# bitlayer-org/tap-stark

Measured on AMD Instinct MI355X. Metric: trace cells/sec (proofs/sec alongside), 2^20x64 BabyBear trace, higher is better.
Workload: dtype u32

## Files before the change

### tap-stark_amd/csrc/kernels.hpp

```cpp
#pragma once
#include <stdint.h>

#include "bb.hpp"
#include "context.hpp"

namespace ts {

struct ColMat {
    uint32_t* d = nullptr;
    uint64_t height = 0;
    uint32_t width = 0;
    uint64_t col_stride = 0;
};

void launch_build_twiddles(Context& ctx, uint32_t* W, uint32_t* Winv, unsigned log_size);
void launch_build_shift_tables(Context& ctx, uint32_t* lo, uint32_t* hi, uint32_t n_hi,
                               uint32_t n_cosets, uint32_t shift_mont, unsigned log_N,
                               unsigned log_blowup, uint32_t scale_mont);
const uint32_t* coset_scale_table(Context& ctx, unsigned log_n, unsigned log_blowup, uint32_t shift);
void launch_transpose_bitrev(Context& ctx, const uint32_t* src, uint32_t* dst, unsigned log_n,
                             uint32_t w, uint64_t dst_col_stride, uint32_t src_width = 0);
bool launch_transpose_bitrev_r16(Context& ctx, const uint32_t* src, uint32_t* dst, unsigned log_n, uint32_t w,
                                 uint64_t dst_col_stride, uint32_t src_width = 0);
void launch_transpose_plain(Context& ctx, const uint32_t* src, uint32_t* dst, uint64_t n, uint32_t w,
                            uint64_t dst_col_stride);
void launch_transpose_to_row_major(Context& ctx, const uint32_t* src, uint64_t col_stride,
                                   uint32_t* dst, uint64_t h, uint32_t w);
void coset_lde(Context& ctx, uint32_t* evals, uint64_t in_col_stride, uint32_t ncols, unsigned log_n,
               unsigned log_blowup, uint32_t shift, uint32_t* out, uint64_t out_col_stride,
               uint32_t beta0 = 0, uint32_t n_beta = 0, bool first_round_done = false,
               uint32_t* evals2 = nullptr, uint32_t shift2 = 0, uint32_t gw = 0);

constexpr int MAX_BATCH_MATS = 64;
struct LeafMats {
    const uint32_t* d[MAX_BATCH_MATS];
    uint64_t col_stride[MAX_BATCH_MATS];
    uint32_t width[MAX_BATCH_MATS];
    uint8_t row_shift[MAX_BATCH_MATS];
    uint32_t n_mats;
    uint32_t total_width;
    const uint32_t* const* cols;
};
void launch_leaf_hash(Context& ctx, const LeafMats& mats, uint64_t height, uint32_t* digests);
void launch_leaf_hash_ef_pairs(Context& ctx, const uint32_t* vec, uint64_t n_rows, uint32_t* digests);
struct DevChallenger;
bool launch_merkle_levels(Context& ctx, uint32_t* tree, unsigned log_leaves,
// ... 48 lines not shown
};
void launch_bary_dots(Context& ctx, const ColMat& m, unsigned log_n, const Ef* weights,
                      uint32_t n_points, Ef* out, BaryPending* pending = nullptr);
void launch_bary_finish(Context& ctx, BaryPending& pending);
struct ReduceArgs {
    Ef z_mont[2];
    Ef off_mont[2];
    Ef rys[2];
    uint32_t n_points;
    uint32_t accumulate;
};
void launch_reduce(Context& ctx, const ColMat& m, unsigned log_h, const uint32_t* d_alpha_pows_mont,
                   const ReduceArgs& args, Ef* ro);
struct FusedReduceArgs {
    Ef z_mont[2];
    Ef off_t[2];
    Ef k0, k1;
    const uint32_t* chunk_w;
    const uint32_t* chunk[MAX_QUOTIENT_CHUNKS];
    uint64_t chunk_stride;
    uint32_t n_chunks;
    uint64_t row0, rows;
};
void launch_reduce_fused(Context& ctx, const ColMat& trace, unsigned log_h,
                         const uint32_t* d_alpha_pows_mont, const FusedReduceArgs& args, Ef* ro);

void launch_fri_fold(Context& ctx, const Ef* in, uint64_t h, Ef beta_canonical, Ef* out,
                     uint32_t* next_digests);
void launch_fri_fold_dev(Context& ctx, const Ef* in, uint64_t h, const Ef* d_beta, Ef* out,
                         uint32_t* next_digests, uint64_t h_global = 0, uint64_t row0 = 0);
// ... 45 lines not shown
```

### tap-stark_amd/csrc/ntt_lde.hip

```cpp
#include "kernels.hpp"

namespace ts {

constexpr int LOG_M = 12;
constexpr int NT_MID = 512;
constexpr int chunk_threads(int lm) { return lm == 14 ? 512 : 256; }
constexpr int TILE_ELEMS = 8192;

__device__ __forceinline__ uint32_t pad(uint32_t i) { return i + (i >> 5); }
constexpr int padded(int n) { return n + (n >> 5); }

template <int K, bool INV, bool TOP>
__device__ __forceinline__ void radix_butterflies(uint32_t (&v)[1 << K], unsigned s_base, unsigned u0,
                                                  uint32_t c, uint32_t hi,
                                                  const uint32_t* __restrict__ W) {
    constexpr int R = 1 << K;
    if (!INV) {
#pragma unroll
        for (int d = 0; d < K; d++) {
            const int half = R >> (d + 1);
            const uint32_t* __restrict__ wp = W + ((1u << (s_base + u0 + d)) + (c << (u0 + d)) + (hi << d));
#pragma unroll
            for (int q = 0; q < R; q++) {
                if ((q & half) == 0) {
// ... 94 lines not shown
template <int NTH>
__device__ __forceinline__ void tile_inverse_rt(uint32_t* s, unsigned log_len, unsigned log_T,
                                                unsigned s_base, uint32_t c,
                                                const uint32_t* __restrict__ Winv) {
    if (log_len == 0) return;
    const unsigned nr = (log_len + 3) / 4, q = log_len / nr, rem = log_len % nr;
    unsigned u = log_len;
    for (int r = (int)nr - 1; r >= 0; r--) {
        const unsigned k = q + ((unsigned)r < rem ? 1u : 0u);
        u -= k;
        radix_round_rt<true, NTH>((int)k, s, log_len + log_T, u, s_base, c, Winv);
    }
}

template <int LM>
__device__ __forceinline__ void chunk_load(uint32_t* s, const uint32_t* __restrict__ g) {
    constexpr int NT = chunk_threads(LM);
    const uint4* g4 = reinterpret_cast<const uint4*>(g);
    uint4 v[(1 << LM) / 4 / NT];
#pragma unroll
    for (int k = 0; k < (1 << LM) / 4 / NT; k++) v[k] = g4[threadIdx.x + (uint32_t)k * NT];
#pragma unroll
    for (int k = 0; k < (1 << LM) / 4 / NT; k++) {
        const uint32_t i4 = threadIdx.x + (uint32_t)k * NT;
        const uint32_t a = 4 * i4 + (i4 >> 3);
        s[a] = v[k].x;
        s[a + 1] = v[k].y;
        s[a + 2] = v[k].z;
        s[a + 3] = v[k].w;
    }
    __syncthreads();
}
template <int LM, bool CANON>
__device__ __forceinline__ void chunk_store(const uint32_t* s, uint32_t* __restrict__ g) {
    constexpr int NT = chunk_threads(LM);
    uint4* g4 = reinterpret_cast<uint4*>(g);
// ... 13 lines not shown
    constexpr int NT = chunk_threads(LM);
    constexpr int K0 = LM == 12 ? 4 : 5;
    constexpr int K1 = LM == 14 ? 5 : 4;
    static_assert(K0 + K1 + 4 == LM, "chunk plan");
    if (!INV) {
        radix_round<K0, false, LM - K0, NT>(s, LM, 0, sb, c, W);
        radix_round<K1, false, 4, NT>(s, LM, K0, sb, c, W);
        radix_round<4, false, 0, NT>(s, LM, K0 + K1, sb, c, W);
    } else {
        if (!SKIP_R16) radix_round<4, true, 0, NT>(s, LM, K0 + K1, sb, c, W);
        radix_round<K1, true, 4, NT>(s, LM, K0, sb, c, W);
        radix_round<K0, true, LM - K0, NT>(s, LM, 0, sb, c, W);
    }
}

template <int LM, bool SKIP_R16 = false>
__global__ void __launch_bounds__(chunk_threads(LM))
k_intt_contig(uint32_t* __restrict__ data, uint64_t col_stride, unsigned log_n,
              const uint32_t* __restrict__ Winv, uint32_t* __restrict__ data2, uint32_t gw) {
    __shared__ uint32_t s[padded(1 << LM)];
    const uint32_t c = blockIdx.x;
    uint32_t* col = blockIdx.y < gw ? data + (uint64_t)blockIdx.y * col_stride
                                    : data2 + (uint64_t)(blockIdx.y - gw) * col_stride;
    uint32_t* g = col + ((uint64_t)c << LM);
    chunk_load<LM>(s, g);
    chunk_rounds<LM, true, SKIP_R16>(s, log_n - LM, c, Winv);
    chunk_store<LM, false>(s, g);
}

__global__ void __launch_bounds__(256)
k_transpose_bitrev_r16(const uint32_t* __restrict__ src, uint32_t* __restrict__ dst, unsigned log_n,
                       uint32_t w, uint64_t dst_col_stride, uint32_t src_width,
                       const uint32_t* __restrict__ Winv) {
    __shared__ uint32_t tile[64][65];
    const uint32_t p0 = blockIdx.x << 6;
    const uint32_t c0 = blockIdx.y * 64;
    const uint32_t tx = threadIdx.x & 63, ty = threadIdx.x >> 6;
    const uint32_t rb = bitrev32(p0, log_n);
    const uint64_t row_step = (uint64_t)src_width << (log_n - 6);
    uint32_t v[16];
// ... 9 lines not shown
#pragma unroll
    for (int q = 0; q < 16; q++) tile[16 * ty + q][tx] = v[q];
    __syncthreads();
    uint32_t t[16];
#pragma unroll
    for (int k = 0; k < 16; k++) t[k] = tile[tx][ty + 4 * k];
    uint32_t* dp = dst + (uint64_t)(c0 + ty) * dst_col_stride + p0 + tx;
#pragma unroll
    for (int k = 0; k < 16; k++)
        if (c0 + ty + 4 * k < w) dp[(uint64_t)(4 * k) * dst_col_stride] = t[k];
}

template <int LM, int CPW = 1>
__global__ void __launch_bounds__(chunk_threads(LM), CPW > 1 ? 4 : 1)
k_lde_fwd_contig(uint32_t* __restrict__ out, uint64_t out_col_stride, unsigned log_n,
                 const uint32_t* __restrict__ W) {
    __shared__ uint32_t s[padded(1 << LM)];
    constexpr int NT = chunk_threads(LM);
    constexpr int NV = (1 << LM) / 4 / NT;
    const uint32_t beta = blockIdx.z;
    uint32_t* col = out + (uint64_t)blockIdx.y * out_col_stride + ((uint64_t)beta << log_n);
    if constexpr (CPW == 1) {
        const uint32_t c = blockIdx.x;
        uint32_t* o = col + ((uint64_t)c << LM);
        chunk_load<LM>(s, o);
        chunk_rounds<LM, false>(s, log_n - LM, c, W);
        chunk_store<LM, true>(s, o);
    } else {
        const uint32_t c0 = blockIdx.x * CPW;
        uint4 v[NV];
        {
            const uint4* g4 = reinterpret_cast<const uint4*>(col + ((uint64_t)c0 << LM));
#pragma unroll
            for (int k = 0; k < NV; k++) v[k] = g4[threadIdx.x + (uint32_t)k * NT];
        }
// ... 16 lines not shown
                for (int k = 0; k < NV; k++) v[k] = g4[threadIdx.x + (uint32_t)k * NT];
            }
            chunk_rounds<LM, false>(s, log_n - LM, c, W);
            chunk_store<LM, true>(s, col + ((uint64_t)c << LM));
            __syncthreads();
        }
    }
}

template <int PLAN, int TILE = TILE_ELEMS, int NTM = NT_MID, int LM = LOG_M>
__global__ void __launch_bounds__(NTM)
k_lde_mid(const uint32_t* __restrict__ evals, uint64_t in_col_stride, uint32_t* __restrict__ out,
          uint64_t out_col_stride, unsigned log_n, unsigned log_len, unsigned log_T,
          unsigned row_shift, unsigned beta0, unsigned n_cosets, const uint32_t* __restrict__ W,
          const uint32_t* __restrict__ Winv, const uint32_t* __restrict__ scale_a,
          const uint32_t* __restrict__ evals2, const uint32_t* __restrict__ scale_b, uint32_t gw) {
    __shared__ uint32_t s[padded(TILE)];
    constexpr int PER_THREAD = TILE / NTM;
    if (PLAN == 1) {
        log_len = 8;
        log_T = 5;
    }
    const bool remap = PLAN == 0 && log_T < 5 && gridDim.x >= 8;
    uint32_t bx = remap ? (blockIdx.x & 7) * (gridDim.x >> 3) + (blockIdx.x >> 3) : blockIdx.x;
    uint32_t col_id = blockIdx.y;
    if constexpr (PLAN == 1) {
        const uint32_t ncols = gridDim.x >> (LM - 5);
        bx = (blockIdx.x & 31) + 32 * (blockIdx.x / (32 * ncols));
        col_id = (blockIdx.x >> 5) % ncols;
    }
    const uint32_t j2_0 = bx << log_T;
    const uint32_t* g = (col_id < gw ? evals + (uint64_t)col_id * in_col_stride
                                     : evals2 + (uint64_t)(col_id - gw) * in_col_stride) + j2_0;
    const uint32_t* __restrict__ scale = col_id < gw ? scale_a : scale_b;
    const uint32_t total = 1u << (log_len + log_T);
    const uint32_t tmask = (1u << log_T) - 1;
    if constexpr (PLAN == 1) {
        uint32_t t[PER_THREAD];
#pragma unroll
        for (int k = 0; k < PER_THREAD; k++) {
            const uint32_t i = threadIdx.x + (uint32_t)k * NTM;
            t[k] = g[((uint64_t)(i >> log_T) << row_shift) + (i & tmask)];
        }
#pragma unroll
        for (int k = 0; k < PER_THREAD; k++) s[pad(threadIdx.x + (uint32_t)k * NTM)] = t[k];
    } else {
        for (uint32_t i = threadIdx.x; i < total; i += NTM)
            s[pad(i)] = g[((uint64_t)(i >> log_T) << row_shift) + (i & tmask)];
    }
    __syncthreads();
    if (PLAN == 1) {
        radix_round<4, true, 5, NTM>(s, 13, 4, 0, 0, Winv);
    } else {
        tile_inverse_rt<NTM>(s, log_len, log_T, 0, 0, Winv);
    }
    uint32_t coef[PER_THREAD];
#pragma unroll
    for (int k = 0; k < PER_THREAD; k++) {
        const uint32_t i = threadIdx.x + (uint32_t)k * NTM;
        coef[k] = i < total ? s[pad(i)] : 0u;
// ... 1 lines not shown
    constexpr int GP = PER_THREAD / 16;
    if constexpr (PLAN == 1) {
#pragma unroll
        for (int j = 0; j < GP; j++) {
            uint32_t v[16];
#pragma unroll
            for (int q = 0; q < 16; q++) v[q] = coef[j + GP * q];
            radix_butterflies<4, true, true>(v, 0, 0, 0, 0, Winv);
#pragma unroll
            for (int q = 0; q < 16; q++) coef[j + GP * q] = v[q];
        }
    }
    constexpr bool PREFETCH = PLAN == 1;
    uint32_t scv[PREFETCH ? 16 : 1];
    const uint32_t* scp = nullptr;
    if constexpr (PREFETCH) {
        const uint32_t i0 = threadIdx.x;
        scp = scale + ((uint64_t)(i0 >> 5) << LM) + (i0 & 31) + j2_0;
#pragma unroll
        for (int q = 0; q < 16; q++)
            scv[q] = (scp + ((uint64_t)beta0 << log_n))[(uint64_t)q * (NTM >> 5) << LM];
    }
    for (uint32_t bl = 0; bl < n_cosets; bl++) {
        const uint32_t beta = beta0 + bl;
        const uint32_t* sc = scale + ((uint64_t)beta << log_n);
        __syncthreads();
        if constexpr (PLAN == 1) {
#pragma unroll
            for (int j = 0; j < GP; j++) {
                uint32_t v[16];
#pragma unroll
                for (int q = 0; q < 16; q++) v[q] = mont_mul_lazy(coef[j + GP * q], scv[q]);
                if (bl + 1 < n_cosets) {
                    const uint32_t* nx = scp + ((uint64_t)(beta + 1) << log_n);
#pragma unroll
                    for (int q = 0; q < 16; q++) scv[q] = nx[(uint64_t)q * (NTM >> 5) << LM];
                }
                radix_butterflies<4, false, true>(v, 0, 0, 0, 0, W);
#pragma unroll
                for (int q = 0; q < 16; q++) s[pad(threadIdx.x + (uint32_t)(j + GP * q) * NTM)] = v[q];
            }
            __syncthreads();
            uint32_t* og = out + (uint64_t)col_id * out_col_stride + ((uint64_t)bl << log_n) + j2_0;
            radix_round<4, false, 5, NTM>(s, 13, 4, 0, 0, W);
            uint32_t t[PER_THREAD];
#pragma unroll
            for (int k = 0; k < PER_THREAD; k++) t[k] = s[pad(threadIdx.x + (uint32_t)k * NTM)];
            uint32_t* ot = og + ((uint64_t)(threadIdx.x >> 5) << LM) + (threadIdx.x & 31);
#pragma unroll
// ... 27 lines not shown
}

bool launch_transpose_bitrev_r16(Context& ctx, const uint32_t* src, uint32_t* dst, unsigned log_n, uint32_t w,
                                 uint64_t dst_col_stride, uint32_t src_width) {
    if (w == 0 || log_n <= lde_chunk_log(log_n)) return false;
    ctx.ensure_twiddles(log_n);
    TS_LAUNCH(ctx, k_transpose_bitrev_r16, dim3(1u << (log_n - 6), (w + 63) / 64), dim3(256), 0, src, dst, log_n, w,
              dst_col_stride, src_width ? src_width : w, (const uint32_t*)ctx.d_twiddle_inv);
    TS_HIP(hipGetLastError());
    return true;
}

void coset_lde(Context& ctx, uint32_t* evals, uint64_t in_col_stride, uint32_t ncols, unsigned log_n,
               unsigned log_blowup, uint32_t shift, uint32_t* out, uint64_t out_col_stride,
               uint32_t beta0, uint32_t n_beta, bool first_round_done, uint32_t* evals2, uint32_t shift2,
               uint32_t gw) {
    if (ncols == 0) return;
    TS_REQUIRE(evals2 == nullptr || (gw >= 1 && gw < ncols && shift2 != 0), TS_ERR_INVALID,
               "coset_lde: second matrix needs its first column and its shift");
    if (evals2 == nullptr) gw = 0xffffffffu;
    TS_REQUIRE(log_n + log_blowup <= 27, TS_ERR_INVALID, "coset_lde: log_n + log_blowup > 27");
    TS_REQUIRE(ncols >= 1 && ncols <= 65535, TS_ERR_INVALID, "coset_lde: bad column count");
    const unsigned LM = lde_chunk_log(log_n);
    TS_REQUIRE(!first_round_done || log_n > LM, TS_ERR_INVARIANT, "coset_lde: no contiguous inverse pass at this size");
    const bool two_pass = log_n > LM;
    const unsigned sA = two_pass ? log_n - LM : 0;
    TS_REQUIRE(sA <= 14, TS_ERR_INVALID, "coset_lde: log_n > 26");
    ctx.ensure_twiddles(log_n == 0 ? 1 : log_n);
    const uint32_t* W = ctx.d_twiddle_fwd;
    const uint32_t* Winv = ctx.d_twiddle_inv;
    unsigned log_T = 0;
    if (two_pass && sA <= 13)
        while ((1u << (sA + log_T + 1)) <= (unsigned)TILE_ELEMS && log_T < 6) log_T++;

    const uint32_t n_cosets = 1u << log_blowup;
    if (n_beta == 0) n_beta = n_cosets - beta0;
    TS_REQUIRE(beta0 < n_cosets && n_beta <= n_cosets - beta0, TS_ERR_INVALID, "coset_lde: coset range");
    const uint32_t* scale = coset_scale_table(ctx, log_n, log_blowup, shift);
    const uint32_t* scale2 = evals2 ? coset_scale_table(ctx, log_n, log_blowup, shift2) : nullptr;

    if (two_pass) {
        TS_REQUIRE(in_col_stride % 4 == 0 && out_col_stride % 4 == 0, TS_ERR_INVALID,
                   "coset_lde: column strides must be multiples of 4 elements");
        if (ctx.lde_pass_mask & 1u) {
            StageTimer t(&ctx, "lde: inverse NTT, contiguous stages");
            const dim3 g(1u << sA, ncols);
#define TS_INTT(LMV)                                                                                          \
    do {                                                                                                      \
        if (first_round_done)                                                                                 \
            TS_LAUNCH(ctx, (k_intt_contig<LMV, true>), g, dim3(chunk_threads(LMV)), 0, evals, in_col_stride, log_n, \
                      Winv, evals2, gw);                                                                      \
        else                                                                                                  \
            TS_LAUNCH(ctx, k_intt_contig<LMV>, g, dim3(chunk_threads(LMV)), 0, evals, in_col_stride, log_n, Winv, \
                      evals2, gw);                                                                            \
    } while (0)
            if (LM == 12) TS_INTT(12);
            else if (LM == 13) TS_INTT(13);
            else TS_INTT(14);
#undef TS_INTT
        }
        StageTimer t_rest(&ctx, "lde: strided pass + forward NTT of the owned cosets");
        const dim3 grid(1u << (LM - log_T), ncols);
        const dim3 grid1((1u << (LM - log_T)) * ncols);
#define TS_MID_ARGS                                                                            \
    (const uint32_t*)evals, in_col_stride, out, out_col_stride, log_n, sA, log_T, (unsigned)LM, \
        beta0, n_beta, W, Winv, scale, (const uint32_t*)evals2, scale2, gw
        if (!(ctx.lde_pass_mask & 2u)) {
        } else if (sA == 14)
            TS_LAUNCH(ctx, (k_lde_mid<0, 16384>), grid, dim3(NT_MID), 0, TS_MID_ARGS);
        else if (sA == 8 && log_T == 5 && LM == 12)
            TS_LAUNCH(ctx, k_lde_mid<1>, grid1, dim3(NT_MID), 0, TS_MID_ARGS);
        else if (sA == 8 && log_T == 5 && LM == 13)
            TS_LAUNCH(ctx, (k_lde_mid<1, 8192, 512, 13>), grid1, dim3(NT_MID), 0, TS_MID_ARGS);
        else if (sA == 8 && log_T == 5 && LM == 14)
            TS_LAUNCH(ctx, (k_lde_mid<1, 8192, 512, 14>), grid1, dim3(NT_MID), 0, TS_MID_ARGS);
        else
            TS_LAUNCH(ctx, k_lde_mid<0>, grid, dim3(NT_MID), 0, TS_MID_ARGS);
        const dim3 gf(1u << sA, ncols, n_beta);
        if (!(ctx.lde_pass_mask & 4u)) {
        } else if (LM == 12)
            TS_LAUNCH(ctx, k_lde_fwd_contig<12>, gf, dim3(chunk_threads(12)), 0, out, out_col_stride, log_n, W);
        else if (LM == 13)
            TS_LAUNCH(ctx, k_lde_fwd_contig<13>, gf, dim3(chunk_threads(13)), 0, out, out_col_stride, log_n, W);
        else
            TS_LAUNCH(ctx, (k_lde_fwd_contig<14, 4>), dim3(gf.x / 4, gf.y, gf.z), dim3(chunk_threads(14)), 0, out,
                      out_col_stride, log_n, W);
    } else {
        TS_LAUNCH(ctx, k_lde_mid<0>, dim3(1, ncols), dim3(NT_MID), 0, (const uint32_t*)evals,
                  in_col_stride, out, out_col_stride, log_n, log_n, 0u, 0u, beta0, n_beta, W, Winv, scale,
                  (const uint32_t*)evals2, scale2, gw);
    }
    TS_HIP(hipGetLastError());
}

}
```

### tap-stark_amd/csrc/open.hip

```cpp
#include "kernels.hpp"

namespace ts {

__device__ __forceinline__ uint32_t root_bitrev(const uint32_t* __restrict__ W, unsigned L, uint64_t r) {
    if (L == 0) return R_MOD_P;
    uint32_t w = W[((uint64_t)1 << (L - 1)) + (r >> 1)];
    return (r & 1) ? neg(w) : w;
}

constexpr int BW_ROWS = 4;

__global__ void __launch_bounds__(256)
k_bary_weights(unsigned log_n, const uint32_t* __restrict__ W, uint32_t gen_mont, Ef z0, Ef z1,
               uint32_t n_points, Ef* __restrict__ out) {
    const uint64_t n = 1ull << log_n;
    const uint64_t t0 = ((uint64_t)blockIdx.x * blockDim.x + threadIdx.x) * BW_ROWS;
    if (t0 >= n) return;
    Ef num[2 * BW_ROWS];
    uint32_t nrm[2 * BW_ROWS], pre[2 * BW_ROWS], xs[BW_ROWS];
    uint32_t run = R_MOD_P;
#pragma unroll
    for (int k = 0; k < BW_ROWS; k++) {
        const bool ok = t0 + k < n;
        uint32_t x = ok ? mont_mul(gen_mont, root_bitrev(W, log_n, t0 + k)) : R_MOD_P;
// ... 184 lines not shown
            TS_LAUNCH(ctx, (k_bary_dots<1, 64>), grid, dim3(256), 0, md, m.col_stride, m.width, log_n,
                      weights, partial.p, rows_per_block);
    }
    TS_HIP(hipGetLastError());
    BaryPending own;
    BaryPending& pend = pending ? *pending : own;
    if (pend.n == 2) launch_bary_finish(ctx, pend);
    pend.partial[pend.n] = std::move(partial);
    pend.out[pend.n] = reinterpret_cast<uint32_t*>(out);
    pend.n_blocks[pend.n] = n_blocks;
    pend.n_words[pend.n] = n_words;
    pend.n++;
    if (!pending) launch_bary_finish(ctx, pend);
}

__device__ __forceinline__ void row_dot_acc(uint64_t (&acc)[4], const uint32_t* __restrict__ m,
                                            uint64_t col_stride, uint32_t width, uint64_t X,
                                            const uint32_t* __restrict__ weights) {
    uint64_t a0 = acc[0], a1 = acc[1], a2 = acc[2], a3 = acc[3];
    constexpr int B = 8;
    const uint32_t* col = m + X;
    uint32_t i = 0;
    for (; i + B <= width; i += B) {
        uint32_t v[B];
#pragma unroll
        for (int k = 0; k < B; k++) v[k] = col[(uint64_t)(i + k) * col_stride];
#pragma unroll
        for (int k = 0; k < B; k++) {
            const uint32_t* ap = weights + 4 * (i + k);
            a0 = lazy_mac(a0, v[k], ap[0]);
            a1 = lazy_mac(a1, v[k], ap[1]);
            a2 = lazy_mac(a2, v[k], ap[2]);
            a3 = lazy_mac(a3, v[k], ap[3]);
            if (k & 1) {
                a0 = lazy_fix(a0);
                a1 = lazy_fix(a1);
                a2 = lazy_fix(a2);
                a3 = lazy_fix(a3);
            }
        }
    }
    if (i < width) {
        uint32_t v[B];
#pragma unroll
        for (int k = 0; k < B; k++) v[k] = i + k < width ? col[(uint64_t)(i + k) * col_stride] : 0u;
#pragma unroll
        for (int k = 0; k < B; k++) {
            if (i + k < width) {
                const uint32_t* ap = weights + 4 * (i + k);
                a0 = lazy_mac(a0, v[k], ap[0]);
                a1 = lazy_mac(a1, v[k], ap[1]);
                a2 = lazy_mac(a2, v[k], ap[2]);
                a3 = lazy_mac(a3, v[k], ap[3]);
            }
            if (k & 1) {
                a0 = lazy_fix(a0);
                a1 = lazy_fix(a1);
                a2 = lazy_fix(a2);
                a3 = lazy_fix(a3);
            }
        }
    }
    acc[0] = a0; acc[1] = a1; acc[2] = a2; acc[3] = a3;
}
__device__ __forceinline__ Ef row_dot_alpha(const uint32_t* __restrict__ m, uint64_t col_stride,
                                            uint32_t width, uint64_t X,
                                            const uint32_t* __restrict__ alpha_pows) {
    uint64_t acc[4] = {0, 0, 0, 0};
    row_dot_acc(acc, m, col_stride, width, X, alpha_pows);
    return Ef{{lazy_finish(acc[0]), lazy_finish(acc[1]), lazy_finish(acc[2]), lazy_finish(acc[3])}};
}

template <int NP>
__device__ __forceinline__ void inv_denoms(uint32_t x_mont, const Ef* z_mont, Ef* out) {
    Ef num[NP];
    uint32_t nrm[NP];
#pragma unroll
    for (int p = 0; p < NP; p++) {
        const Ef z = z_mont[p];
        Ef u = Ef{{sub(x_mont, z.c[0]), neg(z.c[1]), neg(z.c[2]), neg(z.c[3])}};
        ef_inv_parts(u, num[p], nrm[p]);
    }
    if (NP == 2) {
        uint32_t inv = mont_inv(mont_mul(nrm[0], nrm[NP - 1]));
        out[0] = ef_mul_base(num[0], mont_mul(inv, nrm[NP - 1]));
        out[NP - 1] = ef_mul_base(num[NP - 1], mont_mul(inv, nrm[0]));
    } else {
        out[0] = ef_mul_base(num[0], mont_inv(nrm[0]));
    }
}

template <int NP>
__global__ void __launch_bounds__(256)
k_reduce(const uint32_t* __restrict__ m, uint64_t col_stride, uint32_t width, unsigned log_h,
         const uint32_t* __restrict__ W, uint32_t gen_mont, const uint32_t* __restrict__ alpha_pows,
         ReduceArgs args, Ef* __restrict__ ro) {
    const uint64_t h = 1ull << log_h;
    const uint64_t X = (uint64_t)blockIdx.x * blockDim.x + threadIdx.x;
    if (X >= h) return;
    const Ef S = row_dot_alpha(m, col_stride, width, X, alpha_pows);
    const uint32_t x = mont_mul(gen_mont, root_bitrev(W, log_h, X));
    Ef inv_d[NP];
    inv_denoms<NP>(x, args.z_mont, inv_d);
// ... 11 lines not shown
    TS_REQUIRE(args.n_points >= 1 && args.n_points <= 2, TS_ERR_INVALID, "reduce: 1 or 2 points");
    ctx.ensure_twiddles(log_h == 0 ? 1 : log_h);
    const uint64_t h = 1ull << log_h;
    dim3 grid((unsigned)((h + 255) / 256));
    if (args.n_points == 2)
        TS_LAUNCH(ctx, k_reduce<2>, grid, dim3(256), 0, (const uint32_t*)m.d, m.col_stride, m.width,
                  log_h, (const uint32_t*)ctx.d_twiddle_fwd, to_mont(GENERATOR), d_alpha_pows_mont, args,
                  ro);
    else
        TS_LAUNCH(ctx, k_reduce<1>, grid, dim3(256), 0, (const uint32_t*)m.d, m.col_stride, m.width,
                  log_h, (const uint32_t*)ctx.d_twiddle_fwd, to_mont(GENERATOR), d_alpha_pows_mont, args,
                  ro);
    TS_HIP(hipGetLastError());
}

__global__ void __launch_bounds__(256)
k_reduce_fused(const uint32_t* __restrict__ trace, uint64_t trace_stride, uint32_t width,
               unsigned log_h, const uint32_t* __restrict__ W, uint32_t gen_mont,
               const uint32_t* __restrict__ alpha_pows, FusedReduceArgs a, Ef* __restrict__ ro) {
    const uint64_t X = (uint64_t)blockIdx.x * blockDim.x + threadIdx.x;
    if (X >= a.rows) return;
    const Ef St = row_dot_alpha(trace, trace_stride, width, X, alpha_pows);
    const uint32_t x = mont_mul(gen_mont, root_bitrev(W, log_h, a.row0 + X));
    Ef inv_d[2];
    inv_denoms<2>(x, a.z_mont, inv_d);
    uint64_t acc[4] = {0, 0, 0, 0};
    uint32_t c = 0;
    for (; c + 2 <= a.n_chunks; c += 2) {
        uint32_t v[8];
#pragma unroll
        for (int k = 0; k < 8; k++) v[k] = a.chunk[c + (k >> 2)][(uint64_t)(k & 3) * a.chunk_stride + X];
        const uint32_t* ap = a.chunk_w + 16 * c;
#pragma unroll
        for (int k = 0; k < 8; k++) {
#pragma unroll
            for (int j = 0; j < 4; j++) acc[j] = lazy_mac(acc[j], v[k], ap[4 * k + j]);
            if (k & 1) {
#pragma unroll
                for (int j = 0; j < 4; j++) acc[j] = lazy_fix(acc[j]);
            }
        }
    }
    for (; c < a.n_chunks; c++) row_dot_acc(acc, a.chunk[c], a.chunk_stride, 4, X, a.chunk_w + 16 * c);
    const Ef D{{lazy_finish(acc[0]), lazy_finish(acc[1]), lazy_finish(acc[2]), lazy_finish(acc[3])}};
    const Ef g0 = ef_sub(ef_add(ef_mul(St, a.off_t[0]), D), a.k0);
    const Ef g1 = ef_sub(ef_mul(St, a.off_t[1]), a.k1);
    const Ef r = ef_add(ef_mul(g0, inv_d[0]), ef_mul(g1, inv_d[1]));
    *reinterpret_cast<uint4*>(ro + X) = make_uint4(r.c[0], r.c[1], r.c[2], r.c[3]);
}

void launch_reduce_fused(Context& ctx, const ColMat& trace, unsigned log_h,
                         const uint32_t* d_alpha_pows_mont, const FusedReduceArgs& args, Ef* ro) {
    TS_REQUIRE(args.n_chunks <= (uint32_t)MAX_QUOTIENT_CHUNKS, TS_ERR_INVALID, "reduce_fused: too many chunks");
    ctx.ensure_twiddles(log_h == 0 ? 1 : log_h);
    FusedReduceArgs a = args;
    if (a.rows == 0) {
        a.row0 = 0;
        a.rows = 1ull << log_h;
    }
    TS_REQUIRE(a.row0 + a.rows <= (1ull << log_h), TS_ERR_INVALID, "reduce_fused: row range");
    TS_LAUNCH(ctx, k_reduce_fused, dim3((unsigned)((a.rows + 255) / 256)), dim3(256), 0,
              (const uint32_t*)trace.d, trace.col_stride, trace.width, log_h,
              (const uint32_t*)ctx.d_twiddle_fwd, to_mont(GENERATOR), d_alpha_pows_mont, a, ro);
    TS_HIP(hipGetLastError());
}

}
```

### tap-stark_amd/csrc/prover_common.cpp

```cpp
#include <stdlib.h>
#include <string.h>

#include <optional>

#include "prover_internal.hpp"

namespace ts {

void h2d(Context& ctx, void* dst, const void* src, size_t bytes) {
    if (!bytes) return;
    const void* from = bytes <= (1u << 20) ? ctx.stage(src, bytes) : src;
    TS_HIP(hipMemcpyAsync(dst, from, bytes, hipMemcpyHostToDevice, ctx.stream));
}
void d2h_sync(Context& ctx, void* dst, const void* src, size_t bytes) {
    if (bytes) TS_HIP(hipMemcpyAsync(dst, src, bytes, hipMemcpyDeviceToHost, ctx.stream));
    ctx.sync();
}

unsigned log2_strict(uint64_t n) {
    unsigned k = 0;
    while ((1ull << k) < n) k++;
    TS_REQUIRE((1ull << k) == n, TS_ERR_INVALID, "height must be a power of two");
    return k;
}
// ... 78 lines not shown
    auto push_lde = [&](uint32_t* d, uint64_t rows, uint32_t width) {
        ColMat cm;
        cm.d = d;
        cm.height = rows;
        cm.width = width;
        cm.col_stride = rows;
        data.ldes.push_back(cm);
    };

    StageTimer t(&ctx, "coset_lde");
    const bool batched = same_height && evals.size() > 1;
    DevBuf<uint32_t> batch;
    if (batched) batch = DevBuf<uint32_t>(&ctx, total_w * lde_rows(evals[0].height));
    size_t batch_col = 0;
    static const bool pair_knob = [] { const char* e = getenv("TS_LDE_PAIR"); return !e || atoi(e) != 0; }();
    if (allow_pair && pair_knob && batched && evals.size() == 2 && evals[0].width == evals[1].width &&
        evals[0].layout == DeviceMatrix::COL_MAJOR_BITREV && evals[1].layout == DeviceMatrix::COL_MAJOR_BITREV) {
        const uint64_t n = evals[0].height, rows = lde_rows(n);
        const uint32_t w = evals[0].width;
        coset_lde(ctx, evals[0].buf.p, n, 2 * w, log2_strict(n), fri.log_blowup,
                  mul(GENERATOR, inv_canon(domain_shifts[0])), batch.p, rows, beta0, n_beta, false, evals[1].buf.p,
                  mul(GENERATOR, inv_canon(domain_shifts[1])), w);
        for (size_t i = 0; i < 2; i++) {
            push_lde(batch.p + i * (size_t)w * rows, rows, w);
            evals[i].buf.reset();
        }
        data.lde_storage.push_back(std::move(batch));
        return;
    }
    for (size_t i = 0; i < evals.size(); i++) {
        DeviceMatrix& m = evals[i];
        const uint64_t n = m.height, rows = lde_rows(n);
        const unsigned log_n = log2_strict(n);
        DevBuf<uint32_t> colmajor;
        uint32_t* ev = m.buf.p;
        bool r16 = false;
        if (m.layout == DeviceMatrix::ROW_MAJOR) {
// ... 2 lines not shown
            colmajor = DevBuf<uint32_t>(&ctx, (size_t)m.width * n);
            r16 = launch_transpose_bitrev_r16(ctx, m.buf.p, colmajor.p, log_n, m.width, n);
            if (!r16) launch_transpose_bitrev(ctx, m.buf.p, colmajor.p, log_n, m.width, n);
            ev = colmajor.p;
        }
        DevBuf<uint32_t> own;
        uint32_t* lde;
        if (batched) {
            lde = batch.p + batch_col * rows;
            batch_col += m.width;
        } else {
            own = DevBuf<uint32_t>(&ctx, (size_t)m.width * rows);
            lde = own.p;
        }
        coset_lde(ctx, ev, n, m.width, log_n, fri.log_blowup, mul(GENERATOR, inv_canon(domain_shifts[i])), lde,
                  rows, beta0, n_beta, r16);
        push_lde(lde, rows, m.width);
        if (!batched) data.lde_storage.push_back(std::move(own));
        m.buf.reset();
    }
    if (batched) data.lde_storage.push_back(std::move(batch));
}

Statement check_statement(const FriConfig& fri, const AirProgram& air, uint32_t trace_width, uint64_t degree,
                          size_t n_public_values) {
    TS_REQUIRE(trace_width == air.width, TS_ERR_INVALID, "prove: trace width != AIR width");
    TS_REQUIRE(n_public_values == air.n_public, TS_ERR_INVALID, "prove: wrong number of public values");
    Statement s;
    s.log_degree = log2_strict(degree);
    s.lqd = air.log_quotient_degree;
    s.qd = 1u << s.lqd;
// ... 230 lines not shown
```

Baseline: 25.00 billion.

## Skip recomputing LDE coset equal to input domain; process row pairs in fused reduce

In the coset LDE, when some output coset coincides with the original evaluation domain (shift times coset root equals one), the input evaluations are copied straight into that output block during the inverse NTT load. The forward NTT and scaling for that coset are then skipped. Separately, the fused opening-reduce kernel now handles two adjacent rows per thread. The rows share their denominator inverses, taken from x and -x through a single inversion of z^2 - x^2, and their trace loads are vectorised. The cost is more template variants and a more complex coset loop, and the two-row path only runs when alignment and parity conditions hold.

New measurement: 25.17 billion, median of 6. Within noise of the previous version (+0.7%).

```diff
diff --git a/tap-stark_amd/csrc/kernels.hpp b/tap-stark_amd/csrc/kernels.hpp
--- a/tap-stark_amd/csrc/kernels.hpp
+++ b/tap-stark_amd/csrc/kernels.hpp
@@ -29,7 +29,7 @@
 void coset_lde(Context& ctx, uint32_t* evals, uint64_t in_col_stride, uint32_t ncols, unsigned log_n,
                unsigned log_blowup, uint32_t shift, uint32_t* out, uint64_t out_col_stride,
                uint32_t beta0 = 0, uint32_t n_beta = 0, bool first_round_done = false,
-               uint32_t* evals2 = nullptr, uint32_t shift2 = 0, uint32_t gw = 0);
+               uint32_t* evals2 = nullptr, uint32_t shift2 = 0, uint32_t gw = 0, uint32_t known = 0);
 
 constexpr int MAX_BATCH_MATS = 64;
 struct LeafMats {
@@ -108,6 +108,7 @@
                    const ReduceArgs& args, Ef* ro);
 struct FusedReduceArgs {
     Ef z_mont[2];
+    Ef z2_mont[2];
     Ef off_t[2];
     Ef k0, k1;
     const uint32_t* chunk_w;
diff --git a/tap-stark_amd/csrc/ntt_lde.hip b/tap-stark_amd/csrc/ntt_lde.hip
--- a/tap-stark_amd/csrc/ntt_lde.hip
+++ b/tap-stark_amd/csrc/ntt_lde.hip
@@ -6,6 +6,11 @@
 constexpr int NT_MID = 512;
 constexpr int chunk_threads(int lm) { return lm == 14 ? 512 : 256; }
 constexpr int TILE_ELEMS = 8192;
+
+constexpr uint32_t NO_BLOCK = 0xffffffffu;
+struct KnownBlocks {
+    uint32_t a, b;
+};
 
 __device__ __forceinline__ uint32_t pad(uint32_t i) { return i + (i >> 5); }
 constexpr int padded(int n) { return n + (n >> 5); }
@@ -132,12 +137,18 @@
 }
 
 template <int LM>
-__device__ __forceinline__ void chunk_load(uint32_t* s, const uint32_t* __restrict__ g) {
+__device__ __forceinline__ void chunk_load(uint32_t* s, const uint32_t* __restrict__ g,
+                                           uint32_t* __restrict__ raw = nullptr) {
     constexpr int NT = chunk_threads(LM);
     const uint4* g4 = reinterpret_cast<const uint4*>(g);
     uint4 v[(1 << LM) / 4 / NT];
 #pragma unroll
     for (int k = 0; k < (1 << LM) / 4 / NT; k++) v[k] = g4[threadIdx.x + (uint32_t)k * NT];
+    if (raw) {
+        uint4* r4 = reinterpret_cast<uint4*>(raw);
+#pragma unroll
+        for (int k = 0; k < (1 << LM) / 4 / NT; k++) r4[threadIdx.x + (uint32_t)k * NT] = v[k];
+    }
 #pragma unroll
     for (int k = 0; k < (1 << LM) / 4 / NT; k++) {
         const uint32_t i4 = threadIdx.x + (uint32_t)k * NT;
@@ -181,16 +192,24 @@
     }
 }
 
-template <int LM, bool SKIP_R16 = false>
+template <int LM, bool SKIP_R16 = false, bool KNOWN = false>
 __global__ void __launch_bounds__(chunk_threads(LM))
 k_intt_contig(uint32_t* __restrict__ data, uint64_t col_stride, unsigned log_n,
-              const uint32_t* __restrict__ Winv, uint32_t* __restrict__ data2, uint32_t gw) {
+              const uint32_t* __restrict__ Winv, uint32_t* __restrict__ data2, uint32_t gw,
+              uint32_t* __restrict__ out, uint64_t out_col_stride, KnownBlocks kb) {
     __shared__ uint32_t s[padded(1 << LM)];
     const uint32_t c = blockIdx.x;
     uint32_t* col = blockIdx.y < gw ? data + (uint64_t)blockIdx.y * col_stride
                                     : data2 + (uint64_t)(blockIdx.y - gw) * col_stride;
     uint32_t* g = col + ((uint64_t)c << LM);
-    chunk_load<LM>(s, g);
+    if constexpr (KNOWN) {
+        const uint32_t k = blockIdx.y < gw ? kb.a : kb.b;
+        chunk_load<LM>(s, g, k == NO_BLOCK ? nullptr
+                                           : out + (uint64_t)blockIdx.y * out_col_stride + ((uint64_t)k << log_n) +
+                                                 ((uint64_t)c << LM));
+    } else {
+        chunk_load<LM>(s, g);
+    }
     chunk_rounds<LM, true, SKIP_R16>(s, log_n - LM, c, Winv);
     chunk_store<LM, false>(s, g);
 }
@@ -230,11 +249,12 @@
 template <int LM, int CPW = 1>
 __global__ void __launch_bounds__(chunk_threads(LM), CPW > 1 ? 4 : 1)
 k_lde_fwd_contig(uint32_t* __restrict__ out, uint64_t out_col_stride, unsigned log_n,
-                 const uint32_t* __restrict__ W) {
+                 const uint32_t* __restrict__ W, uint32_t gw, KnownBlocks kb) {
     __shared__ uint32_t s[padded(1 << LM)];
     constexpr int NT = chunk_threads(LM);
     constexpr int NV = (1 << LM) / 4 / NT;
     const uint32_t beta = blockIdx.z;
+    if (beta == (blockIdx.y < gw ? kb.a : kb.b)) return;
     uint32_t* col = out + (uint64_t)blockIdx.y * out_col_stride + ((uint64_t)beta << log_n);
     if constexpr (CPW == 1) {
         const uint32_t c = blockIdx.x;
@@ -281,7 +301,8 @@
           uint64_t out_col_stride, unsigned log_n, unsigned log_len, unsigned log_T,
           unsigned row_shift, unsigned beta0, unsigned n_cosets, const uint32_t* __restrict__ W,
           const uint32_t* __restrict__ Winv, const uint32_t* __restrict__ scale_a,
-          const uint32_t* __restrict__ evals2, const uint32_t* __restrict__ scale_b, uint32_t gw) {
+          const uint32_t* __restrict__ evals2, const uint32_t* __restrict__ scale_b, uint32_t gw,
+          KnownBlocks known) {
     __shared__ uint32_t s[padded(TILE)];
     constexpr int PER_THREAD = TILE / NTM;
     if (PLAN == 1) {
@@ -300,6 +321,7 @@
     const uint32_t* g = (col_id < gw ? evals + (uint64_t)col_id * in_col_stride
                                      : evals2 + (uint64_t)(col_id - gw) * in_col_stride) + j2_0;
     const uint32_t* __restrict__ scale = col_id < gw ? scale_a : scale_b;
+    const uint32_t kb = col_id < gw ? known.a : known.b;
     const uint32_t total = 1u << (log_len + log_T);
     const uint32_t tmask = (1u << log_T) - 1;
     if constexpr (PLAN == 1) {
@@ -311,6 +333,9 @@
         }
 #pragma unroll
         for (int k = 0; k < PER_THREAD; k++) s[pad(threadIdx.x + (uint32_t)k * NTM)] = t[k];
+    } else if (row_shift == 0 && kb != NO_BLOCK) {
+        uint32_t* ok = out + (uint64_t)col_id * out_col_stride + ((uint64_t)kb << log_n);
+        for (uint32_t i = threadIdx.x; i < total; i += NTM) s[pad(i)] = ok[i] = g[i];
     } else {
         for (uint32_t i = threadIdx.x; i < total; i += NTM)
             s[pad(i)] = g[((uint64_t)(i >> log_T) << row_shift) + (i & tmask)];
@@ -342,14 +367,18 @@
     constexpr bool PREFETCH = PLAN == 1;
     uint32_t scv[PREFETCH ? 16 : 1];
     const uint32_t* scp = nullptr;
+    const uint32_t bl0 = kb == 0 ? 1u : 0u;
     if constexpr (PREFETCH) {
         const uint32_t i0 = threadIdx.x;
         scp = scale + ((uint64_t)(i0 >> 5) << LM) + (i0 & 31) + j2_0;
-#pragma unroll
-        for (int q = 0; q < 16; q++)
-            scv[q] = (scp + ((uint64_t)beta0 << log_n))[(uint64_t)q * (NTM >> 5) << LM];
-    }
-    for (uint32_t bl = 0; bl < n_cosets; bl++) {
+        if (bl0 < n_cosets) {
+#pragma unroll
+            for (int q = 0; q < 16; q++)
+                scv[q] = (scp + ((uint64_t)(beta0 + bl0) << log_n))[(uint64_t)q * (NTM >> 5) << LM];
+        }
+    }
+    for (uint32_t bl = bl0, bl_next; bl < n_cosets; bl = bl_next) {
+        bl_next = bl + 1 == kb ? bl + 2 : bl + 1;
         const uint32_t beta = beta0 + bl;
         const uint32_t* sc = scale + ((uint64_t)beta << log_n);
         __syncthreads();
@@ -359,8 +388,8 @@
                 uint32_t v[16];
 #pragma unroll
                 for (int q = 0; q < 16; q++) v[q] = mont_mul_lazy(coef[j + GP * q], scv[q]);
-                if (bl + 1 < n_cosets) {
-                    const uint32_t* nx = scp + ((uint64_t)(beta + 1) << log_n);
+                if (bl_next < n_cosets) {
+                    const uint32_t* nx = scp + ((uint64_t)(beta0 + bl_next) << log_n);
 #pragma unroll
                     for (int q = 0; q < 16; q++) scv[q] = nx[(uint64_t)q * (NTM >> 5) << LM];
                 }
@@ -418,7 +447,7 @@
 void coset_lde(Context& ctx, uint32_t* evals, uint64_t in_col_stride, uint32_t ncols, unsigned log_n,
                unsigned log_blowup, uint32_t shift, uint32_t* out, uint64_t out_col_stride,
                uint32_t beta0, uint32_t n_beta, bool first_round_done, uint32_t* evals2, uint32_t shift2,
-               uint32_t gw) {
+               uint32_t gw, uint32_t known) {
     if (ncols == 0) return;
     TS_REQUIRE(evals2 == nullptr || (gw >= 1 && gw < ncols && shift2 != 0), TS_ERR_INVALID,
                "coset_lde: second matrix needs its first column and its shift");
@@ -442,6 +471,18 @@
     TS_REQUIRE(beta0 < n_cosets && n_beta <= n_cosets - beta0, TS_ERR_INVALID, "coset_lde: coset range");
     const uint32_t* scale = coset_scale_table(ctx, log_n, log_blowup, shift);
     const uint32_t* scale2 = evals2 ? coset_scale_table(ctx, log_n, log_blowup, shift2) : nullptr;
+    auto known_block = [&](uint32_t sh) {
+        const uint32_t w = two_adic_generator(log_n + log_blowup);
+        for (uint32_t bl = 0; bl < n_beta; bl++)
+            if (mul(sh, pow_canon(w, bitrev32(beta0 + bl, log_blowup))) == 1) return bl;
+        return NO_BLOCK;
+    };
+    KnownBlocks kb{NO_BLOCK, NO_BLOCK};
+    if (!first_round_done) {
+        if (known & 1u) kb.a = known_block(shift);
+        if (evals2 && (known & 2u)) kb.b = known_block(shift2);
+    }
+    const bool any_known = kb.a != NO_BLOCK || kb.b != NO_BLOCK;
 
     if (two_pass) {
         TS_REQUIRE(in_col_stride % 4 == 0 && out_col_stride % 4 == 0, TS_ERR_INVALID,
@@ -449,26 +490,28 @@
         if (ctx.lde_pass_mask & 1u) {
             StageTimer t(&ctx, "lde: inverse NTT, contiguous stages");
             const dim3 g(1u << sA, ncols);
+#define TS_INTT_ARGS evals, in_col_stride, log_n, Winv, evals2, gw, out, out_col_stride, kb
 #define TS_INTT(LMV)                                                                                          \
     do {                                                                                                      \
         if (first_round_done)                                                                                 \
-            TS_LAUNCH(ctx, (k_intt_contig<LMV, true>), g, dim3(chunk_threads(LMV)), 0, evals, in_col_stride, log_n, \
-                      Winv, evals2, gw);                                                                      \
+            TS_LAUNCH(ctx, (k_intt_contig<LMV, true>), g, dim3(chunk_threads(LMV)), 0, TS_INTT_ARGS);         \
+        else if (any_known)                                                                                   \
+            TS_LAUNCH(ctx, (k_intt_contig<LMV, false, true>), g, dim3(chunk_threads(LMV)), 0, TS_INTT_ARGS);  \
         else                                                                                                  \
-            TS_LAUNCH(ctx, k_intt_contig<LMV>, g, dim3(chunk_threads(LMV)), 0, evals, in_col_stride, log_n, Winv, \
-                      evals2, gw);                                                                            \
+            TS_LAUNCH(ctx, k_intt_contig<LMV>, g, dim3(chunk_threads(LMV)), 0, TS_INTT_ARGS);                 \
     } while (0)
             if (LM == 12) TS_INTT(12);
             else if (LM == 13) TS_INTT(13);
             else TS_INTT(14);
 #undef TS_INTT
+#undef TS_INTT_ARGS
         }
         StageTimer t_rest(&ctx, "lde: strided pass + forward NTT of the owned cosets");
         const dim3 grid(1u << (LM - log_T), ncols);
         const dim3 grid1((1u << (LM - log_T)) * ncols);
 #define TS_MID_ARGS                                                                            \
     (const uint32_t*)evals, in_col_stride, out, out_col_stride, log_n, sA, log_T, (unsigned)LM, \
-        beta0, n_beta, W, Winv, scale, (const uint32_t*)evals2, scale2, gw
+        beta0, n_beta, W, Winv, scale, (const uint32_t*)evals2, scale2, gw, kb
         if (!(ctx.lde_pass_mask & 2u)) {
         } else if (sA == 14)
             TS_LAUNCH(ctx, (k_lde_mid<0, 16384>), grid, dim3(NT_MID), 0, TS_MID_ARGS);
@@ -483,16 +526,16 @@
         const dim3 gf(1u << sA, ncols, n_beta);
         if (!(ctx.lde_pass_mask & 4u)) {
         } else if (LM == 12)
-            TS_LAUNCH(ctx, k_lde_fwd_contig<12>, gf, dim3(chunk_threads(12)), 0, out, out_col_stride, log_n, W);
+            TS_LAUNCH(ctx, k_lde_fwd_contig<12>, gf, dim3(chunk_threads(12)), 0, out, out_col_stride, log_n, W, gw, kb);
         else if (LM == 13)
-            TS_LAUNCH(ctx, k_lde_fwd_contig<13>, gf, dim3(chunk_threads(13)), 0, out, out_col_stride, log_n, W);
+            TS_LAUNCH(ctx, k_lde_fwd_contig<13>, gf, dim3(chunk_threads(13)), 0, out, out_col_stride, log_n, W, gw, kb);
         else
             TS_LAUNCH(ctx, (k_lde_fwd_contig<14, 4>), dim3(gf.x / 4, gf.y, gf.z), dim3(chunk_threads(14)), 0, out,
-                      out_col_stride, log_n, W);
+                      out_col_stride, log_n, W, gw, kb);
     } else {
         TS_LAUNCH(ctx, k_lde_mid<0>, dim3(1, ncols), dim3(NT_MID), 0, (const uint32_t*)evals,
                   in_col_stride, out, out_col_stride, log_n, log_n, 0u, 0u, beta0, n_beta, W, Winv, scale,
-                  (const uint32_t*)evals2, scale2, gw);
+                  (const uint32_t*)evals2, scale2, gw, kb);
     }
     TS_HIP(hipGetLastError());
 }
diff --git a/tap-stark_amd/csrc/open.hip b/tap-stark_amd/csrc/open.hip
--- a/tap-stark_amd/csrc/open.hip
+++ b/tap-stark_amd/csrc/open.hip
@@ -222,79 +222,118 @@
     if (!pending) launch_bary_finish(ctx, pend);
 }
 
-__device__ __forceinline__ void row_dot_acc(uint64_t (&acc)[4], const uint32_t* __restrict__ m,
+template <int R>
+__device__ __forceinline__ void load_rows(uint32_t (&v)[R], const uint32_t* __restrict__ p) {
+    if constexpr (R == 2) {
+        const uint2 t = *reinterpret_cast<const uint2*>(p);
+        v[0] = t.x;
+        v[1] = t.y;
+    } else {
+        v[0] = *p;
+    }
+}
+template <int R>
+__device__ __forceinline__ void row_dot_acc(uint64_t (&acc)[R][4], const uint32_t* __restrict__ m,
                                             uint64_t col_stride, uint32_t width, uint64_t X,
                                             const uint32_t* __restrict__ weights) {
-    uint64_t a0 = acc[0], a1 = acc[1], a2 = acc[2], a3 = acc[3];
     constexpr int B = 8;
     const uint32_t* col = m + X;
     uint32_t i = 0;
     for (; i + B <= width; i += B) {
-        uint32_t v[B];
-#pragma unroll
-        for (int k = 0; k < B; k++) v[k] = col[(uint64_t)(i + k) * col_stride];
+        uint32_t v[B][R];
+#pragma unroll
+        for (int k = 0; k < B; k++) load_rows<R>(v[k], col + (uint64_t)(i + k) * col_stride);
 #pragma unroll
         for (int k = 0; k < B; k++) {
             const uint32_t* ap = weights + 4 * (i + k);
-            a0 = lazy_mac(a0, v[k], ap[0]);
-            a1 = lazy_mac(a1, v[k], ap[1]);
-            a2 = lazy_mac(a2, v[k], ap[2]);
-            a3 = lazy_mac(a3, v[k], ap[3]);
-            if (k & 1) {
-                a0 = lazy_fix(a0);
-                a1 = lazy_fix(a1);
-                a2 = lazy_fix(a2);
-                a3 = lazy_fix(a3);
+#pragma unroll
+            for (int r = 0; r < R; r++) {
+#pragma unroll
+                for (int j = 0; j < 4; j++) acc[r][j] = lazy_mac(acc[r][j], v[k][r], ap[j]);
+                if (k & 1) {
+#pragma unroll
+                    for (int j = 0; j < 4; j++) acc[r][j] = lazy_fix(acc[r][j]);
+                }
             }
         }
     }
     if (i < width) {
-        uint32_t v[B];
-#pragma unroll
-        for (int k = 0; k < B; k++) v[k] = i + k < width ? col[(uint64_t)(i + k) * col_stride] : 0u;
+        uint32_t v[B][R];
 #pragma unroll
         for (int k = 0; k < B; k++) {
             if (i + k < width) {
-                const uint32_t* ap = weights + 4 * (i + k);
-                a0 = lazy_mac(a0, v[k], ap[0]);
-                a1 = lazy_mac(a1, v[k], ap[1]);
-                a2 = lazy_mac(a2, v[k], ap[2]);
-                a3 = lazy_mac(a3, v[k], ap[3]);
-            }
-            if (k & 1) {
-                a0 = lazy_fix(a0);
-                a1 = lazy_fix(a1);
-                a2 = lazy_fix(a2);
-                a3 = lazy_fix(a3);
-            }
-        }
-    }
-    acc[0] = a0; acc[1] = a1; acc[2] = a2; acc[3] = a3;
+                load_rows<R>(v[k], col + (uint64_t)(i + k) * col_stride);
+            } else {
+#pragma unroll
+                for (int r = 0; r < R; r++) v[k][r] = 0u;
+            }
+        }
+#pragma unroll
+        for (int k = 0; k < B; k++) {
+#pragma unroll
+            for (int r = 0; r < R; r++) {
+                if (i + k < width) {
+                    const uint32_t* ap = weights + 4 * (i + k);
+#pragma unroll
+                    for (int j = 0; j < 4; j++) acc[r][j] = lazy_mac(acc[r][j], v[k][r], ap[j]);
+                }
+                if (k & 1) {
+#pragma unroll
+                    for (int j = 0; j < 4; j++) acc[r][j] = lazy_fix(acc[r][j]);
+                }
+            }
+        }
+    }
+}
+__device__ __forceinline__ Ef lazy_finish_ef(const uint64_t (&acc)[4]) {
+    return Ef{{lazy_finish(acc[0]), lazy_finish(acc[1]), lazy_finish(acc[2]), lazy_finish(acc[3])}};
 }
 __device__ __forceinline__ Ef row_dot_alpha(const uint32_t* __restrict__ m, uint64_t col_stride,
                                             uint32_t width, uint64_t X,
                                             const uint32_t* __restrict__ alpha_pows) {
-    uint64_t acc[4] = {0, 0, 0, 0};
-    row_dot_acc(acc, m, col_stride, width, X, alpha_pows);
-    return Ef{{lazy_finish(acc[0]), lazy_finish(acc[1]), lazy_finish(acc[2]), lazy_finish(acc[3])}};
-}
-
+    uint64_t acc[1][4] = {{0, 0, 0, 0}};
+    row_dot_acc<1>(acc, m, col_stride, width, X, alpha_pows);
+    return lazy_finish_ef(acc[0]);
+}
+
+__device__ __forceinline__ void ef_inv_two(Ef u0, Ef u1, Ef& i0, Ef& i1) {
+    Ef num0, num1;
+    uint32_t nrm0, nrm1;
+    ef_inv_parts(u0, num0, nrm0);
+    ef_inv_parts(u1, num1, nrm1);
+    const uint32_t inv = mont_inv(mont_mul(nrm0, nrm1));
+    i0 = ef_mul_base(num0, mont_mul(inv, nrm1));
+    i1 = ef_mul_base(num1, mont_mul(inv, nrm0));
+}
 template <int NP>
 __device__ __forceinline__ void inv_denoms(uint32_t x_mont, const Ef* z_mont, Ef* out) {
-    Ef num[NP];
-    uint32_t nrm[NP];
+    Ef u[NP];
 #pragma unroll
     for (int p = 0; p < NP; p++) {
         const Ef z = z_mont[p];
-        Ef u = Ef{{sub(x_mont, z.c[0]), neg(z.c[1]), neg(z.c[2]), neg(z.c[3])}};
-        ef_inv_parts(u, num[p], nrm[p]);
-    }
-    if (NP == 2) {
-        uint32_t inv = mont_inv(mont_mul(nrm[0], nrm[NP - 1]));
-        out[0] = ef_mul_base(num[0], mont_mul(inv, nrm[NP - 1]));
-        out[NP - 1] = ef_mul_base(num[NP - 1], mont_mul(inv, nrm[0]));
+        u[p] = Ef{{sub(x_mont, z.c[0]), neg(z.c[1]), neg(z.c[2]), neg(z.c[3])}};
+    }
+    if constexpr (NP == 2) {
+        ef_inv_two(u[0], u[1], out[0], out[1]);
     } else {
-        out[0] = ef_mul_base(num[0], mont_inv(nrm[0]));
+        Ef num;
+        uint32_t nrm;
+        ef_inv_parts(u[0], num, nrm);
+        out[0] = ef_mul_base(num, mont_inv(nrm));
+    }
+}
+__device__ __forceinline__ void inv_denoms_pair(uint32_t x_mont, const Ef* z_mont, const Ef* z2_mont, Ef* pos,
+                                                Ef* neg_) {
+    const uint32_t xx = mont_mul(x_mont, x_mont);
+    Ef d[2], e[2];
+#pragma unroll
+    for (int p = 0; p < 2; p++) d[p] = Ef{{sub(z2_mont[p].c[0], xx), z2_mont[p].c[1], z2_mont[p].c[2], z2_mont[p].c[3]}};
+    ef_inv_two(d[0], d[1], e[0], e[1]);
+#pragma unroll
+    for (int p = 0; p < 2; p++) {
+        const Ef ze = ef_mul(z_mont[p], e[p]), xe = ef_mul_base(e[p], x_mont);
+        pos[p] = ef_neg(ef_add(xe, ze));
+        neg_[p] = ef_sub(xe, ze);
     }
 }
 
@@ -336,39 +375,58 @@
     TS_HIP(hipGetLastError());
 }
 
+template <int R>
 __global__ void __launch_bounds__(256)
 k_reduce_fused(const uint32_t* __restrict__ trace, uint64_t trace_stride, uint32_t width,
                unsigned log_h, const uint32_t* __restrict__ W, uint32_t gen_mont,
                const uint32_t* __restrict__ alpha_pows, FusedReduceArgs a, Ef* __restrict__ ro) {
-    const uint64_t X = (uint64_t)blockIdx.x * blockDim.x + threadIdx.x;
+    const uint64_t X = ((uint64_t)blockIdx.x * blockDim.x + threadIdx.x) * R;
     if (X >= a.rows) return;
-    const Ef St = row_dot_alpha(trace, trace_stride, width, X, alpha_pows);
+    uint64_t acc[R][4];
+#pragma unroll
+    for (int r = 0; r < R; r++)
+#pragma unroll
+        for (int j = 0; j < 4; j++) acc[r][j] = 0;
+    row_dot_acc<R>(acc, trace, trace_stride, width, X, alpha_pows);
+    Ef St[R];
+#pragma unroll
+    for (int r = 0; r < R; r++) St[r] = lazy_finish_ef(acc[r]);
     const uint32_t x = mont_mul(gen_mont, root_bitrev(W, log_h, a.row0 + X));
-    Ef inv_d[2];
-    inv_denoms<2>(x, a.z_mont, inv_d);
-    uint64_t acc[4] = {0, 0, 0, 0};
+    Ef inv_d[R][2];
+    if constexpr (R == 2) inv_denoms_pair(x, a.z_mont, a.z2_mont, inv_d[0], inv_d[1]);
+    else inv_denoms<2>(x, a.z_mont, inv_d[0]);
+#pragma unroll
+    for (int r = 0; r < R; r++)
+#pragma unroll
+        for (int j = 0; j < 4; j++) acc[r][j] = 0;
     uint32_t c = 0;
     for (; c + 2 <= a.n_chunks; c += 2) {
-        uint32_t v[8];
-#pragma unroll
-        for (int k = 0; k < 8; k++) v[k] = a.chunk[c + (k >> 2)][(uint64_t)(k & 3) * a.chunk_stride + X];
+        uint32_t v[8][R];
+#pragma unroll
+        for (int k = 0; k < 8; k++) load_rows<R>(v[k], a.chunk[c + (k >> 2)] + (uint64_t)(k & 3) * a.chunk_stride + X);
         const uint32_t* ap = a.chunk_w + 16 * c;
 #pragma unroll
         for (int k = 0; k < 8; k++) {
 #pragma unroll
-            for (int j = 0; j < 4; j++) acc[j] = lazy_mac(acc[j], v[k], ap[4 * k + j]);
-            if (k & 1) {
-#pragma unroll
-                for (int j = 0; j < 4; j++) acc[j] = lazy_fix(acc[j]);
-            }
-        }
-    }
-    for (; c < a.n_chunks; c++) row_dot_acc(acc, a.chunk[c], a.chunk_stride, 4, X, a.chunk_w + 16 * c);
-    const Ef D{{lazy_finish(acc[0]), lazy_finish(acc[1]), lazy_finish(acc[2]), lazy_finish(acc[3])}};
-    const Ef g0 = ef_sub(ef_add(ef_mul(St, a.off_t[0]), D), a.k0);
-    const Ef g1 = ef_sub(ef_mul(St, a.off_t[1]), a.k1);
-    const Ef r = ef_add(ef_mul(g0, inv_d[0]), ef_mul(g1, inv_d[1]));
-    *reinterpret_cast<uint4*>(ro + X) = make_uint4(r.c[0], r.c[1], r.c[2], r.c[3]);
+            for (int r = 0; r < R; r++) {
+#pragma unroll
+                for (int j = 0; j < 4; j++) acc[r][j] = lazy_mac(acc[r][j], v[k][r], ap[4 * k + j]);
+                if (k & 1) {
+#pragma unroll
+                    for (int j = 0; j < 4; j++) acc[r][j] = lazy_fix(acc[r][j]);
+                }
+            }
+        }
+    }
+    for (; c < a.n_chunks; c++) row_dot_acc<R>(acc, a.chunk[c], a.chunk_stride, 4, X, a.chunk_w + 16 * c);
+#pragma unroll
+    for (int r = 0; r < R; r++) {
+        const Ef D = lazy_finish_ef(acc[r]);
+        const Ef g0 = ef_sub(ef_add(ef_mul(St[r], a.off_t[0]), D), a.k0);
+        const Ef g1 = ef_sub(ef_mul(St[r], a.off_t[1]), a.k1);
+        const Ef v = ef_add(ef_mul(g0, inv_d[r][0]), ef_mul(g1, inv_d[r][1]));
+        *reinterpret_cast<uint4*>(ro + X + r) = make_uint4(v.c[0], v.c[1], v.c[2], v.c[3]);
+    }
 }
 
 void launch_reduce_fused(Context& ctx, const ColMat& trace, unsigned log_h,
@@ -381,9 +439,16 @@
         a.rows = 1ull << log_h;
     }
     TS_REQUIRE(a.row0 + a.rows <= (1ull << log_h), TS_ERR_INVALID, "reduce_fused: row range");
-    TS_LAUNCH(ctx, k_reduce_fused, dim3((unsigned)((a.rows + 255) / 256)), dim3(256), 0,
-              (const uint32_t*)trace.d, trace.col_stride, trace.width, log_h,
-              (const uint32_t*)ctx.d_twiddle_fwd, to_mont(GENERATOR), d_alpha_pows_mont, a, ro);
+    for (int p = 0; p < 2; p++) a.z2_mont[p] = ef_mul(a.z_mont[p], a.z_mont[p]);
+    bool pairs = a.row0 % 2 == 0 && a.rows % 2 == 0 && trace.col_stride % 2 == 0 && a.chunk_stride % 2 == 0 &&
+                 (uintptr_t)trace.d % 8 == 0;
+    for (uint32_t c = 0; c < a.n_chunks; c++) pairs = pairs && (uintptr_t)a.chunk[c] % 8 == 0;
+#define TS_REDUCE_ARGS                                                                   \
+    (const uint32_t*)trace.d, trace.col_stride, trace.width, log_h, (const uint32_t*)ctx.d_twiddle_fwd, \
+        to_mont(GENERATOR), d_alpha_pows_mont, a, ro
+    if (pairs) TS_LAUNCH(ctx, k_reduce_fused<2>, dim3((unsigned)((a.rows / 2 + 255) / 256)), dim3(256), 0, TS_REDUCE_ARGS);
+    else TS_LAUNCH(ctx, k_reduce_fused<1>, dim3((unsigned)((a.rows + 255) / 256)), dim3(256), 0, TS_REDUCE_ARGS);
+#undef TS_REDUCE_ARGS
     TS_HIP(hipGetLastError());
 }
 
diff --git a/tap-stark_amd/csrc/prover_common.cpp b/tap-stark_amd/csrc/prover_common.cpp
--- a/tap-stark_amd/csrc/prover_common.cpp
+++ b/tap-stark_amd/csrc/prover_common.cpp
@@ -116,13 +116,15 @@
     if (batched) batch = DevBuf<uint32_t>(&ctx, total_w * lde_rows(evals[0].height));
     size_t batch_col = 0;
     static const bool pair_knob = [] { const char* e = getenv("TS_LDE_PAIR"); return !e || atoi(e) != 0; }();
+    const char* known_env = getenv("TS_LDE_KNOWN");
+    const uint64_t known_knob = known_env ? strtoull(known_env, nullptr, 0) : ~0ull;
     if (allow_pair && pair_knob && batched && evals.size() == 2 && evals[0].width == evals[1].width &&
         evals[0].layout == DeviceMatrix::COL_MAJOR_BITREV && evals[1].layout == DeviceMatrix::COL_MAJOR_BITREV) {
         const uint64_t n = evals[0].height, rows = lde_rows(n);
         const uint32_t w = evals[0].width;
         coset_lde(ctx, evals[0].buf.p, n, 2 * w, log2_strict(n), fri.log_blowup,
                   mul(GENERATOR, inv_canon(domain_shifts[0])), batch.p, rows, beta0, n_beta, false, evals[1].buf.p,
-                  mul(GENERATOR, inv_canon(domain_shifts[1])), w);
+                  mul(GENERATOR, inv_canon(domain_shifts[1])), w, (uint32_t)(known_knob & 3u));
         for (size_t i = 0; i < 2; i++) {
             push_lde(batch.p + i * (size_t)w * rows, rows, w);
             evals[i].buf.reset();
@@ -155,7 +157,7 @@
             lde = own.p;
         }
         coset_lde(ctx, ev, n, m.width, log_n, fri.log_blowup, mul(GENERATOR, inv_canon(domain_shifts[i])), lde,
-                  rows, beta0, n_beta, r16);
+                  rows, beta0, n_beta, r16, nullptr, 0, 0, (uint32_t)(known_knob >> i & 1u));
         push_lde(lde, rows, m.width);
         if (!batched) data.lde_storage.push_back(std::move(own));
         m.buf.reset();
```
